# bebop/poly

Measured on AMD Instinct MI355X. Metric: mash.Sketch k-mers hashed/s, higher is better.
Workload: dtype u32

## Files before the change

### poly_amd/csrc/mash_sketch.hip

```cpp
#include <hip/hip_runtime.h>

#include <algorithm>

#include "common.h"
#include "host_pipeline.h"
#include "multi_device.h"
#include <memory>
#include <string>
#include <vector>

#ifndef PH_WPE
#define PH_WPE 6
#endif
#ifndef PH_CAPK
#define PH_CAPK 12u
#endif
#ifndef PH_ABL
#define PH_ABL 0
#endif
#ifndef PH_SEL_ATOMIC
#define PH_SEL_ATOMIC 0
#endif
#ifndef PH_BS_WIN
#define PH_BS_WIN 4
#endif
#ifndef PH_BS_U
#define PH_BS_U 4
#endif
#ifndef PH_SLAB_SIG
#define PH_SLAB_SIG 6u
#endif
#ifndef PH_SLAB_CW
#define PH_SLAB_CW 6u
#endif
#ifndef PH_SLAB_CF
#define PH_SLAB_CF 0u
#endif
#ifndef PH_SLAB_WPE
#define PH_SLAB_WPE 8
#endif

namespace polyhip {
namespace k1 {

constexpr int THREADS = 256;
constexpr int WAVES = THREADS / 64;
#ifndef PH_WTW
#define PH_WTW 512
#endif
constexpr int WTW = PH_WTW;
constexpr int TW = WTW * WAVES;
constexpr int GROUPS = WTW / (4 * 64);
constexpr int NB = 2048;
constexpr uint32_t MARK0 = 0xFFFFFFFFu, MARK1 = 0u;
constexpr int GBATCH = 32;
constexpr uint32_t WL_POSITIONAL = 0x80000000u;
constexpr uint32_t C1 = 0xcc9e2d51u, C2 = 0x1b873593u;

__device__ __forceinline__ uint32_t rotl32(uint32_t x, int r) { return (x << r) | (x >> (32 - r)); }

__device__ __forceinline__ uint32_t premix(uint32_t k)
{
    k *= C1;
    k = rotl32(k, 15);
    k *= C2;
    return k;
}

__device__ __forceinline__ uint32_t chain(uint32_t h) { return rotl32(h, 13) * 5u + 0xe6546b64u; }

__device__ __forceinline__ uint32_t fmix32(uint32_t h)
{
    h ^= h >> 16;
    h *= 0x85ebca6bu;
    h ^= h >> 13;
    h *= 0xc2b2ae35u;
    h ^= h >> 16;
    return h;
}

__device__ __forceinline__ uint32_t funnel_bytes(uint32_t hi, uint32_t lo, uint32_t sh)
{
    return __builtin_amdgcn_alignbyte(hi, lo, sh);
}

__device__ __forceinline__ uint32_t wave_incl_scan(uint32_t v)
{
    v += (uint32_t)__builtin_amdgcn_update_dpp(0, (int)v, 0x111, 0xF, 0xF, true);
    v += (uint32_t)__builtin_amdgcn_update_dpp(0, (int)v, 0x112, 0xF, 0xF, true);
    v += (uint32_t)__builtin_amdgcn_update_dpp(0, (int)v, 0x114, 0xF, 0xF, true);
    v += (uint32_t)__builtin_amdgcn_update_dpp(0, (int)v, 0x118, 0xF, 0xF, true);
    v += (uint32_t)__builtin_amdgcn_update_dpp(0, (int)v, 0x142, 0xA, 0xF, false);
    v += (uint32_t)__builtin_amdgcn_update_dpp(0, (int)v, 0x143, 0xC, 0xF, false);
    return v;
}

struct Smem {
    uint32_t *seqb;
    uint32_t *P;
    uint32_t *cand;
    uint32_t *binned;
    uint32_t *misc;
    uint32_t *lut;
    uint32_t *bins;
    uint32_t *biglist;
    uint32_t listcap;
};

constexpr uint32_t BIG_BIN = 32;
constexpr uint32_t BIG_LIST_CAP = 512;

template <class Bin, class Emit>
__device__ __attribute__((noinline)) void rank_big_bins(const uint32_t *__restrict__ binned, const Bin *__restrict__ bins,
                                              const uint32_t *__restrict__ biglist, uint32_t nbig, uint32_t s, Emit emit)
{
    const int lane = threadIdx.x & 63, wave = threadIdx.x >> 6;
    const uint64_t below = (1ull << lane) - 1ull;
    for (uint32_t q = wave; q < nbig; q += WAVES) {
        const uint32_t b = biglist[q];
        const uint32_t st = b ? bins[b - 1] : 0u, en = bins[b];
        uint32_t base = st, lastv = 0;
        bool first = true;
        while (base < s && base < en) {
            uint32_t m = 0xFFFFFFFFu;
            bool has = false;
            for (uint32_t x = st + lane; x < en; x += 64) {
                const uint32_t o = binned[x];
                if (first || o > lastv) {
                    m = min(m, o);
                    has = true;
                }
            }
            if (__ballot(has) == 0ull)
                break;
#pragma unroll
            for (int d = 32; d >= 1; d >>= 1)
                m = min(m, (uint32_t)__shfl_xor((int)m, d, 64));
            for (uint32_t x0 = st; x0 < en; x0 += 64) {
                const uint32_t x = x0 + lane;
                const bool eq = x < en && binned[x] == m;
                const uint64_t mask = __ballot(eq);
                const uint32_t pos = base + (uint32_t)__builtin_popcountll(mask & below);
                if (eq && pos < s)
                    emit(pos, m);
                base += (uint32_t)__builtin_popcountll(mask);
            }
            lastv = m;
            first = false;
        }
    }
}

template <class ForEach>
__device__ uint32_t bottom_s(const Smem &sm, uint32_t s, uint32_t tau, uint32_t binned_cap, bool keep_partial,
                             ForEach for_each)
{
    const int tid = threadIdx.x;
    uint32_t *bins = sm.P;
    const int sig = 32 - __builtin_clz(tau | 1u);
    const int shift = sig > 11 ? sig - 11 : 0;
    __syncthreads();

    for (int b = tid; b < NB; b += THREADS)
        bins[b] = 0;
    if (tid == 0)
        sm.misc[8] = 0;
    __syncthreads();
    for_each([&](uint32_t h) {
        if (h <= tau)
            atomicAdd(&bins[h >> shift], 1u);
    });
    __syncthreads();

    {
        uint32_t v[8], sum = 0;
#pragma unroll
        for (int i = 0; i < 8; ++i) {
            v[i] = bins[8 * tid + i];
            sum += v[i];
        }
        uint32_t incl = sum;
#pragma unroll
        for (int d = 1; d < 64; d <<= 1) {
            uint32_t t = __shfl_up(incl, d, 64);
            if ((tid & 63) >= d)
                incl += t;
        }
        if ((tid & 63) == 63)
            sm.misc[4 + (tid >> 6)] = incl;
        __syncthreads();
        uint32_t run = incl - sum;
        for (int w = 0; w < (tid >> 6); ++w)
            run += sm.misc[4 + w];
#pragma unroll
        for (int i = 0; i < 8; ++i) {
            bins[8 * tid + i] = run;
            run += v[i];
            if (v[i] > BIG_BIN) {
                const uint32_t slot = atomicAdd(&sm.misc[8], 1u);
                if (slot < BIG_LIST_CAP)
                    sm.seqb[slot] = (uint32_t)(8 * tid + i);
            }
        }
        if (tid == THREADS - 1)
            sm.misc[3] = run;
    }
    __syncthreads();
    const uint32_t T = sm.misc[3];
    if (T > binned_cap || (T < s && !keep_partial))
        return T;
    for_each([&](uint32_t h) {
        if (h <= tau)
            sm.binned[atomicAdd(&bins[h >> shift], 1u)] = h;
    });
    __syncthreads();
    if (T < s) {
        for (uint32_t j = tid; j < T; j += THREADS)
            sm.cand[j] = sm.binned[j];
        __syncthreads();
        if (tid == 0)
            sm.misc[0] = T;
        __syncthreads();
        return T;
    }
    const uint32_t nbig = sm.misc[8];
    const bool by_waves = nbig <= BIG_LIST_CAP;
    for (uint32_t j = tid; j < T; j += THREADS) {
        const uint32_t h = sm.binned[j];
        const uint32_t b = h >> shift;
        const uint32_t start = b ? bins[b - 1] : 0u;
        if (start >= s)
            continue;
        const uint32_t end = bins[b];
        if (by_waves && end - start > BIG_BIN)
            continue;
        uint32_t rank = 0;
        for (uint32_t x = start; x < end; ++x) {
            const uint32_t o = sm.binned[x];
            rank += (o < h) || (o == h && x < j);
        }
        const uint32_t pos = start + rank;
        if (pos < s)
            sm.cand[pos] = h;
    }
    if (by_waves && nbig)
        rank_big_bins(sm.binned, bins, sm.seqb, nbig, s, [cand = sm.cand](uint32_t pos, uint32_t h) { cand[pos] = h; });
    __syncthreads();
    if (tid == 0) {
        sm.misc[0] = s;
        sm.misc[1] = sm.cand[s - 1];
    }
    __syncthreads();
    return T;
}

__device__ __forceinline__ void wave_sync()
{
    asm volatile("" ::: "memory");
    __builtin_amdgcn_wave_barrier();
    asm volatile("" ::: "memory");
}

template <int KS> struct Stager {
    static constexpr int NI = KS > 0 ? ((WTW / 4 + KS / 4 + 2 + 3) + 63) / 64 : 1;
    uint32_t lo[NI], hi[NI];

    __device__ __forceinline__ static void fetch(const uint32_t *__restrict__ gdw, uint32_t gsh, int64_t gbytes,
                                                 int64_t gi, bool full, uint32_t &l, uint32_t &h)
    {
        if (PH_ABL == 6) {
            l = (uint32_t)gi * 0x9E3779B9u;
            h = l;
            return;
        }
        h = 0u;
        if (full) {
            l = gdw[gi];
            if (gsh)
                h = gdw[gi + 1];
        } else {
            l = (gi * 4 < gbytes) ? gdw[gi] : 0u;
            if (gsh)
                h = ((gi + 1) * 4 < gbytes) ? gdw[gi + 1] : 0u;
        }
    }

    __device__ __forceinline__ void load(const uint32_t *__restrict__ gdw, uint32_t gsh, int64_t gbytes, int64_t t0,
                                         uint32_t n_seq_dw, bool full)
    {
        if (KS > 0) {
            const int64_t dbase = t0 >> 2;
#pragma unroll
            for (int i = 0; i < NI; ++i) {
                const uint32_t d = (threadIdx.x & 63) + i * 64;
                if (d < n_seq_dw)
                    fetch(gdw, gsh, gbytes, dbase + d, full, lo[i], hi[i]);
            }
        }
    }

    __device__ __forceinline__ void store(uint32_t *__restrict__ seqb, const uint32_t *__restrict__ gdw, uint32_t gsh,
                                          int64_t gbytes, int64_t t0, uint32_t n_seq_dw, bool full)
    {
        if (KS > 0) {
#pragma unroll
            for (int i = 0; i < NI; ++i) {
                const uint32_t d = (threadIdx.x & 63) + i * 64;
                if (d < n_seq_dw)
                    seqb[d] = gsh ? funnel_bytes(hi[i], lo[i], gsh) : lo[i];
            }
        } else {
            const int64_t dbase = t0 >> 2;
            for (uint32_t d = threadIdx.x & 63; d < n_seq_dw; d += 64) {
                uint32_t l, h;
                fetch(gdw, gsh, gbytes, dbase + d, full, l, h);
                seqb[d] = gsh ? funnel_bytes(h, l, gsh) : l;
            }
        }
    }
};

template <int KS, class Emit>
__device__ __forceinline__ void tile_compute(const uint32_t *__restrict__ seqb, uint32_t *__restrict__ P,
                                             const uint32_t *__restrict__ lut, uint32_t k, Emit emit)
{
    const int lane = threadIdx.x & 63;
    const int nblk = (int)(k >> 2);
    const int tail = (int)(k & 3);
    const uint32_t tailmask = tail == 0 ? 0u : (0xFFFFFFFFu >> (32 - 8 * tail));

    {
        const int nq = (WTW >> 2) + nblk;
        for (int q = lane; q < (PH_ABL == 1 ? 0 : nq); q += 64) {
            const uint32_t d0 = seqb[q], d1 = seqb[q + 1];
            uint4 p;
            p.x = premix(d0);
            p.y = premix(funnel_bytes(d1, d0, 1));
            p.z = premix(funnel_bytes(d1, d0, 2));
            p.w = premix(funnel_bytes(d1, d0, 3));
            reinterpret_cast<uint4 *>(P)[q] = p;
        }
    }
    wave_sync();

    const uint4 *P4 = reinterpret_cast<const uint4 *>(P);
#pragma unroll
    for (int g = 0; g < GROUPS; ++g) {
        const int wq = lane + 64 * g;
        uint32_t h[4] = {0u, 0u, 0u, 0u};
        if (KS > 0) {
#pragma unroll
            for (int j = 0; j < (PH_ABL == 2 ? 1 : (KS >> 2)); ++j) {
                const uint4 p = P4[wq + j];
                h[0] = chain(h[0] ^ p.x);
                h[1] = chain(h[1] ^ p.y);
                h[2] = chain(h[2] ^ p.z);
                h[3] = chain(h[3] ^ p.w);
            }
        } else {
            for (int j = 0; j < nblk; ++j) {
                const uint4 p = P4[wq + j];
                h[0] = chain(h[0] ^ p.x);
                h[1] = chain(h[1] ^ p.y);
                h[2] = chain(h[2] ^ p.z);
                h[3] = chain(h[3] ^ p.w);
            }
        }
        if (PH_ABL == 3) {
        } else if (tail == 1) {
            const uint32_t tb = seqb[wq + nblk];
            h[0] ^= lut[tb & 0xFFu];
            h[1] ^= lut[(tb >> 8) & 0xFFu];
            h[2] ^= lut[(tb >> 16) & 0xFFu];
            h[3] ^= lut[tb >> 24];
        } else if (tail) {
            const uint32_t d0 = seqb[wq + nblk], d1 = seqb[wq + nblk + 1];
            h[0] ^= premix(d0 & tailmask) ^ k;
            h[1] ^= premix(funnel_bytes(d1, d0, 1) & tailmask) ^ k;
            h[2] ^= premix(funnel_bytes(d1, d0, 2) & tailmask) ^ k;
            h[3] ^= premix(funnel_bytes(d1, d0, 3) & tailmask) ^ k;
        } else {
#pragma unroll
            for (int c = 0; c < 4; ++c)
                h[c] ^= k;
        }
#pragma unroll
        for (int c = 0; c < 4; ++c)
            h[c] = PH_ABL == 3 ? h[c] : fmix32(h[c]);
        emit(4u * (uint32_t)wq, h);
    }
    wave_sync();
}

template <int KS, bool LOCKSTEP, class Before, class EmitFull, class EmitPart>
__device__ __forceinline__ void run_tiles(const Smem &sm, const uint32_t *__restrict__ gdw, uint32_t gsh,
                                          int64_t gbytes, int64_t nwin, uint32_t k, uint32_t n_seq_dw, uint32_t n_P_w,
                                          Before before, EmitFull emit_full, EmitPart emit_part)
{
    const int wave = threadIdx.x >> 6;
    uint32_t *seqb = sm.seqb + wave * n_seq_dw;
    uint32_t *P = sm.P + wave * n_P_w;
    const int64_t stage_bytes = (int64_t)n_seq_dw * 4 + 4;
    auto is_full = [&](int64_t t0) { return (nwin - t0) >= (int64_t)WTW && t0 + stage_bytes <= gbytes; };
    Stager<KS> st;
    const int64_t first = (int64_t)wave * WTW;
    if (first < nwin)
        st.load(gdw, gsh, gbytes, first, n_seq_dw, is_full(first));
    for (int64_t T0 = 0; T0 < nwin; T0 += TW) {
        if (LOCKSTEP)
            before(T0);
        const int64_t t0 = T0 + first;
        if (t0 >= nwin)
            continue;
        const bool full = is_full(t0);
        st.store(seqb, gdw, gsh, gbytes, t0, n_seq_dw, full);
        wave_sync();
        if (t0 + TW < nwin)
            st.load(gdw, gsh, gbytes, t0 + TW, n_seq_dw, is_full(t0 + TW));
        if (full) {
            tile_compute<KS>(seqb, P, sm.lut, k, [&](uint32_t w0, const uint32_t(&h)[4]) { emit_full(t0, w0, h, 4u); });
        } else {
            const uint32_t wl = (uint32_t)((nwin - t0) < (int64_t)WTW ? (nwin - t0) : (int64_t)WTW);
            tile_compute<KS>(seqb, P, sm.lut, k, [&](uint32_t w0, const uint32_t(&h)[4]) {
                emit_part(t0, w0, h, w0 >= wl ? 0u : (wl - w0 < 4u ? wl - w0 : 4u));
            });
        }
    }
}

__device__ __forceinline__ void append4(uint32_t *__restrict__ counter, uint32_t *__restrict__ cand, uint32_t cap,
                                        const uint32_t (&h)[4], uint32_t nvalid, uint32_t tau)
{
    bool a[4];
    uint64_t m[4];
    uint32_t cnt[4], total = 0;
#pragma unroll
    for (int c = 0; c < 4; ++c) {
        a[c] = (PH_ABL == 4 ? h[c] == 12345u : h[c] <= tau) && (uint32_t)c < nvalid;
        m[c] = __ballot(a[c]);
        cnt[c] = (uint32_t)__popcll(m[c]);
        total += cnt[c];
    }
    if (total == 0)
        return;
    uint32_t base = 0;
    if ((threadIdx.x & 63) == 0)
        base = atomicAdd(counter, total);
    base = __builtin_amdgcn_readfirstlane(base);
#pragma unroll
    for (int c = 0; c < 4; ++c) {
        if (a[c]) {
            const uint32_t idx = base + __builtin_amdgcn_mbcnt_hi((uint32_t)(m[c] >> 32),
                                                                  __builtin_amdgcn_mbcnt_lo((uint32_t)m[c], 0u));
            if (idx < cap)
                cand[idx] = h[c];
        }
        base += cnt[c];
    }
}

constexpr int BSU = PH_BS_U;
constexpr uint32_t BS_MARGIN = (PH_BS_WIN + 3u) & ~3u;
#define BS_SYNC()              \
    do {                       \
        if (PH_ABL != 21)      \
            __syncthreads();   \
    } while (0)
template <bool FIN>
__device__ void bottom_s_fast(const Smem &sm, uint32_t s, uint32_t tau, uint32_t C, uint32_t nbf_log2,
                              uint32_t *__restrict__ outp, const uint32_t *__restrict__ src, uint32_t first,
                              uint32_t step, uint32_t cnt)
{
    const int tid = threadIdx.x;
    auto fin = [](uint32_t h) { return FIN ? h ^ (h >> 16) : h; };
    uint32_t *bins = sm.bins;
    const uint16_t *bins16 = reinterpret_cast<const uint16_t *>(bins);
    const int sig = 32 - __builtin_clz(tau | 1u);
    const int shift = sig > (int)nbf_log2 ? sig - (int)nbf_log2 : 0;
    auto one = [](uint32_t b) { return 1u << ((b & 1u) << 4); };
    const bool wide = nbf_log2 == 11u;
    if (wide)
        reinterpret_cast<uint4 *>(bins)[tid] = make_uint4(0, 0, 0, 0);
    else
        reinterpret_cast<uint2 *>(bins)[tid] = make_uint2(0, 0);
    if (tid == 0)
        sm.misc[8] = 0;
    if (PH_BS_WIN) {
        if (tid < PH_BS_WIN)
            sm.binned[-1 - tid] = 0u;
        else if (tid < 2 * PH_BS_WIN)
            sm.binned[C + (uint32_t)tid - PH_BS_WIN] = 0xFFFFFFFFu;
    }
    BS_SYNC();
    for (uint32_t i0 = first; i0 < cnt; i0 += BSU * step) {
        uint32_t h[BSU];
#pragma unroll
        for (int u = 0; u < BSU; ++u)
            h[u] = i0 + u * step < cnt ? fin(src[i0 + u * step]) : 0u;
#pragma unroll
        for (int u = 0; u < BSU; ++u)
            if (i0 + u * step < cnt) {
                const uint32_t b = h[u] >> shift;
                atomicAdd(&bins[b >> 1], one(b));
            }
    }
    BS_SYNC();
    {
        uint32_t w[4];
        if (wide) {
            const uint4 t = reinterpret_cast<const uint4 *>(bins)[tid];
            w[0] = t.x, w[1] = t.y, w[2] = t.z, w[3] = t.w;
        } else {
            const uint2 t = reinterpret_cast<const uint2 *>(bins)[tid];
            w[0] = t.x, w[1] = t.y, w[2] = 0u, w[3] = 0u;
        }
        uint32_t c[8], sum = 0;
#pragma unroll
        for (int i = 0; i < 8; ++i) {
            c[i] = (w[i >> 1] >> (16 * (i & 1))) & 0xFFFFu;
            sum += c[i];
        }
        const uint32_t incl = wave_incl_scan(sum);
        if ((tid & 63) == 63)
            sm.misc[4 + (tid >> 6)] = incl;
        BS_SYNC();
        uint32_t run = incl - sum;
        for (int w8 = 0; w8 < (tid >> 6); ++w8)
            run += sm.misc[4 + w8];
        const uint32_t b0 = (uint32_t)tid << (wide ? 3 : 2);
#pragma unroll
        for (int i = 0; i < 4; ++i) {
            w[i] = run | ((run + c[2 * i]) << 16);
            run += c[2 * i] + c[2 * i + 1];
        }
        if (wide)
            reinterpret_cast<uint4 *>(bins)[tid] = make_uint4(w[0], w[1], w[2], w[3]);
        else
            reinterpret_cast<uint2 *>(bins)[tid] = make_uint2(w[0], w[1]);
        if (max(max(max(c[0], c[1]), max(c[2], c[3])), max(max(c[4], c[5]), max(c[6], c[7]))) > BIG_BIN) {
#pragma unroll
            for (int i = 0; i < 8; ++i)
                if (c[i] > BIG_BIN) {
                    const uint32_t slot = atomicAdd(&sm.misc[8], 1u);
                    if (slot < sm.listcap)
                        sm.biglist[slot] = b0 + (uint32_t)i;
                }
        }
    }
    BS_SYNC();
    for (uint32_t i0 = first; i0 < cnt; i0 += BSU * step) {
        uint32_t h[BSU], at[BSU];
#pragma unroll
        for (int u = 0; u < BSU; ++u)
            h[u] = i0 + u * step < cnt ? fin(src[i0 + u * step]) : 0u;
#pragma unroll
        for (int u = 0; u < BSU; ++u)
            if (i0 + u * step < cnt) {
                const uint32_t b = h[u] >> shift;
                at[u] = (atomicAdd(&bins[b >> 1], one(b)) >> ((b & 1u) << 4)) & 0xFFFFu;
            }
#pragma unroll
        for (int u = 0; u < BSU; ++u)
            if (i0 + u * step < cnt)
                sm.binned[at[u]] = h[u];
    }
    BS_SYNC();
    const uint32_t nbig = sm.misc[8];
    const bool by_waves = nbig <= sm.listcap;
    auto rank_in_bin = [&](uint32_t j, uint32_t hv) {
        const uint32_t b = hv >> shift;
        const uint32_t start = b ? bins16[b - 1] : 0u, end = bins16[b];
        if (start >= s || (by_waves && end - start > BIG_BIN))
            return;
        uint32_t pos = start;
        for (uint32_t x = start; x < end; ++x) {
            const uint32_t o = sm.binned[x];
            pos += (o < hv) || (o == hv && x < j);
        }
        if (pos < s)
            outp[pos] = hv;
    };
#if PH_BS_WIN
    if (PH_ABL != 22) {
        const uint32_t lim = 1u << shift;
        for (uint32_t j = tid; j < C; j += THREADS) {
            const uint32_t *__restrict__ w = sm.binned + j;
            const uint32_t hv = w[0];
            uint32_t pos = j;
            bool far;
            {
                uint32_t l[PH_BS_WIN], r[PH_BS_WIN];
#pragma unroll
                for (int d = 0; d < PH_BS_WIN; ++d) {
                    l[d] = w[-1 - d];
                    r[d] = w[1 + d];
                }
#pragma unroll
                for (int d = 0; d < PH_BS_WIN; ++d) {
                    pos -= l[d] > hv ? 1u : 0u;
                    pos += r[d] < hv ? 1u : 0u;
                }
                far = ((l[PH_BS_WIN - 1] ^ hv) < lim) | ((r[PH_BS_WIN - 1] ^ hv) < lim);
            }
            if (__builtin_expect(far, 0))
                rank_in_bin(j, hv);
            else if (pos < s)
                outp[pos] = hv;
        }
    }
#else
    for (uint32_t j = tid; j < C; j += THREADS)
        rank_in_bin(j, sm.binned[j]);
#endif
    if (by_waves && nbig)
        rank_big_bins(sm.binned, bins16, sm.biglist, nbig, s, [outp](uint32_t pos, uint32_t hv) { outp[pos] = hv; });
}

struct ReadView {
    const uint32_t *gdw;
    uint32_t gsh;
    int64_t gbytes, nwin;
};

__device__ __forceinline__ ReadView view(const uint8_t *__restrict__ seqs, const uint64_t *__restrict__ offs,
                                         uint64_t r, uint32_t k)
{
    ReadView v;
    const uint64_t o0 = offs[r], o1 = offs[r + 1];
    const int64_t n = (int64_t)(o1 - o0);
    v.nwin = n - (int64_t)k;
    v.gsh = (uint32_t)((uintptr_t)(seqs + o0) & 3);
    v.gdw = reinterpret_cast<const uint32_t *>(seqs + o0 - v.gsh);
    v.gbytes = n + v.gsh;
    return v;
}

template <int KS>
__global__ __launch_bounds__(THREADS) __attribute__((amdgpu_waves_per_eu(PH_WPE, 8))) void sketch_fast_kernel(const uint8_t *__restrict__ seqs,
                                                             const uint64_t *__restrict__ offs, uint64_t nseq,
                                                             uint32_t k_rt, uint32_t s, uint32_t *__restrict__ out,
                                                             uint32_t n_seq_dw, uint32_t n_P_w, uint32_t n_P,
                                                             uint32_t capf, uint32_t nbf_log2)
{
    extern __shared__ __attribute__((aligned(16))) uint32_t smem_raw[];
    Smem sm;
    sm.seqb = smem_raw;
    sm.P = sm.seqb + WAVES * n_seq_dw;
    sm.cand = sm.P + n_P;
    sm.binned = sm.cand + capf + BS_MARGIN;
    sm.misc = sm.binned + capf + BS_MARGIN;
    sm.lut = sm.misc + 16;
    sm.bins = sm.P;
    sm.biglist = sm.seqb;
    sm.listcap = BIG_LIST_CAP;

    const uint32_t k = KS > 0 ? (uint32_t)KS : k_rt;
    const int tid = threadIdx.x;
    sm.lut[tid] = premix((uint32_t)tid) ^ k;
    auto nothing = [](int64_t) {};

    for (uint64_t r = blockIdx.x; r < nseq; r += gridDim.x) {
        const ReadView rv = view(seqs, offs, r, k);
        if (rv.nwin <= 0)
            continue;
        uint32_t *__restrict__ outp = out + r * (uint64_t)s;

        if (rv.nwin < (int64_t)s) {
            __syncthreads();
            auto put = [&](int64_t t0, uint32_t w0, const uint32_t(&h)[4], uint32_t nvalid) {
#pragma unroll
                for (int c = 0; c < 4; ++c)
                    if ((uint32_t)c < nvalid)
                        outp[t0 + w0 + c] = h[c];
            };
            run_tiles<KS, false>(sm, rv.gdw, rv.gsh, rv.gbytes, rv.nwin, k, n_seq_dw, n_P_w, nothing, put, put);
            continue;
        }

        uint32_t tau0 = 0xFFFFFFFFu;
        {
            const uint64_t target = (uint64_t)s + 6ull * (uint64_t)__builtin_sqrtf((float)s) + 16ull;
            if ((int64_t)target < rv.nwin)
                tau0 = (uint32_t)((target << 32) / (uint64_t)rv.nwin);
        }
        bool ok = tau0 != 0xFFFFFFFFu || rv.nwin <= (int64_t)capf;
        __syncthreads();
        if (tid == 0)
            sm.misc[0] = 0;
        __syncthreads();
        uint32_t C = 0;
        if (ok) {
            auto keep = [&](int64_t, uint32_t, const uint32_t(&h)[4], uint32_t nvalid) {
                append4(&sm.misc[0], sm.cand, capf, h, nvalid, tau0);
            };
            run_tiles<KS, false>(sm, rv.gdw, rv.gsh, rv.gbytes, rv.nwin, k, n_seq_dw, n_P_w, nothing, keep, keep);
            __syncthreads();
            C = sm.misc[0];
            ok = C >= s && C <= capf;
        }
        if (ok) {
            if (PH_ABL == 5) {
                for (uint32_t i = tid; i < s; i += THREADS)
                    outp[i] = sm.cand[i];
            } else {
                bottom_s_fast<false>(sm, s, tau0, C, nbf_log2, outp, sm.cand, (uint32_t)tid, THREADS, C);
            }
        } else if (tid == 0) {
            outp[0] = MARK0;
            outp[1] = MARK1;
        }
    }
}

template <int KS> struct Slabs {
    static constexpr int NBLK = KS >> 2, TAIL = KS & 3;
    static constexpr int DUPD = NBLK + 2;
    const uint32_t *__restrict__ gdw;
    uint32_t gsh;
    uint32_t *__restrict__ seqb;
    uint32_t *__restrict__ P;
    const uint32_t *__restrict__ lut;
    int lane;

    uint32_t u_inside;
    uint32_t gb32;
    __device__ __forceinline__ void gload(uint32_t u, uint32_t &lo, uint32_t &hi) const
    {
        const uint32_t *__restrict__ slab = gdw + (uint64_t)u * 64;
        hi = 0u;
        if (__builtin_expect(u < u_inside, 1)) {
            lo = slab[lane];
            if (gsh)
                hi = slab[lane + 1];
        } else {
            const int left = (int)(gb32 - u * 256u);
            lo = lane * 4 < left ? slab[lane] : 0u;
            if (gsh)
                hi = (lane + 1) * 4 < left ? slab[lane + 1] : 0u;
        }
    }

    template <int PAR> __device__ __forceinline__ void stage(uint32_t lo, uint32_t hi) const
    {
        const uint32_t v = gsh ? funnel_bytes(hi, lo, gsh) : lo;
        seqb[1 + 64 * PAR + lane] = v;
        if (PAR == 0) {
            if (lane < DUPD)
                seqb[129 + lane] = v;
        } else if (lane == 63) {
            seqb[0] = v;
        }
    }

    template <int PAR> __device__ __forceinline__ void premix_unit() const
    {
        const uint32_t d0 = seqb[64 * PAR + lane], d1 = seqb[64 * PAR + lane + 1];
        uint4 p;
        p.x = premix(d0);
        p.y = premix(funnel_bytes(d1, d0, 1));
        p.z = premix(funnel_bytes(d1, d0, 2));
        p.w = premix(funnel_bytes(d1, d0, 3));
        uint4 *P4 = reinterpret_cast<uint4 *>(P);
        if (PAR == 0) {
            P4[(lane + 127) & 127] = p;
            if (lane >= 1 && lane <= NBLK)
                P4[127 + lane] = p;
        } else {
            P4[63 + lane] = p;
        }
    }

    template <int PAR> __device__ __forceinline__ void hash(uint32_t (&h)[4]) const
    {
        const uint4 *b = reinterpret_cast<const uint4 *>(P) + 64 * PAR + lane;
        h[0] = h[1] = h[2] = h[3] = 0u;
#pragma unroll
        for (int j = 0; j < (PH_ABL == 16 ? 1 : NBLK); ++j) {
            const uint4 p = b[j];
            h[0] = chain(h[0] ^ p.x);
            h[1] = chain(h[1] ^ p.y);
            h[2] = chain(h[2] ^ p.z);
            h[3] = chain(h[3] ^ p.w);
        }
        const uint32_t *t = seqb + 1 + 64 * PAR + lane + NBLK;
        if (TAIL == 1) {
            const uint32_t tb = t[0];
            uint32_t off[4];
            const uint32_t two = 2u;
            asm("v_lshlrev_b32_sdwa %0, %1, %2 dst_sel:DWORD dst_unused:UNUSED_PAD src0_sel:DWORD src1_sel:BYTE_0" : "=v"(off[0]) : "v"(two), "v"(tb));
            asm("v_lshlrev_b32_sdwa %0, %1, %2 dst_sel:DWORD dst_unused:UNUSED_PAD src0_sel:DWORD src1_sel:BYTE_1" : "=v"(off[1]) : "v"(two), "v"(tb));
            asm("v_lshlrev_b32_sdwa %0, %1, %2 dst_sel:DWORD dst_unused:UNUSED_PAD src0_sel:DWORD src1_sel:BYTE_2" : "=v"(off[2]) : "v"(two), "v"(tb));
            asm("v_lshlrev_b32_sdwa %0, %1, %2 dst_sel:DWORD dst_unused:UNUSED_PAD src0_sel:DWORD src1_sel:BYTE_3" : "=v"(off[3]) : "v"(two), "v"(tb));
#pragma unroll
            for (int c = 0; c < 4; ++c)
                h[c] ^= *reinterpret_cast<const __attribute__((address_space(3))) uint32_t *>((uintptr_t)off[c]);
        } else if (TAIL) {
            constexpr uint32_t tailmask = 0xFFFFFFFFu >> (32 - 8 * (TAIL ? TAIL : 1));
            const uint32_t d0 = t[0], d1 = t[1];
            h[0] ^= premix(d0 & tailmask) ^ (uint32_t)KS;
            h[1] ^= premix(funnel_bytes(d1, d0, 1) & tailmask) ^ (uint32_t)KS;
            h[2] ^= premix(funnel_bytes(d1, d0, 2) & tailmask) ^ (uint32_t)KS;
            h[3] ^= premix(funnel_bytes(d1, d0, 3) & tailmask) ^ (uint32_t)KS;
        } else {
#pragma unroll
            for (int c = 0; c < 4; ++c)
                h[c] ^= (uint32_t)KS;
        }
#pragma unroll
        for (int c = 0; c < 4; ++c) {
            uint32_t x = h[c];
            if (PH_ABL != 17) {
                x ^= x >> 16;
                x *= 0x85ebca6bu;
                x ^= x >> 13;
            }
            x *= 0xc2b2ae35u;
            h[c] = x;
        }
    }
};

template <bool PARTIAL>
__device__ __forceinline__ void append_own(uint32_t *__restrict__ seg, uint32_t capw, uint32_t &cnt, const uint32_t (&h)[4],
                                           uint32_t nvalid, uint32_t tauq)
{
    bool a[4];
    uint64_t m[4];
    uint32_t n[4], total = 0;
#pragma unroll
    for (int c = 0; c < 4; ++c) {
        a[c] = h[c] <= tauq && (!PARTIAL || (uint32_t)c < nvalid);
        m[c] = __ballot(a[c]);
        n[c] = (uint32_t)__popcll(m[c]);
        total += n[c];
    }
    uint32_t base = __builtin_amdgcn_readfirstlane(cnt);
    cnt = base + total;
#if PH_SEL_ATOMIC
    {
        uint32_t *ctr = seg + capw;
        uint32_t slot[4];
#pragma unroll
        for (int c = 0; c < 4; ++c)
            if (a[c])
                slot[c] = atomicInc(ctr, capw - 1u);
#pragma unroll
        for (int c = 0; c < 4; ++c)
            if (a[c])
                seg[slot[c]] = h[c];
        return;
    }
#endif
    if (cnt <= capw) {
#pragma unroll
        for (int c = 0; c < 4; ++c) {
            uint32_t *__restrict__ at = seg + base;
            if (a[c])
                at[__builtin_amdgcn_mbcnt_hi((uint32_t)(m[c] >> 32), __builtin_amdgcn_mbcnt_lo((uint32_t)m[c], 0u))] = h[c];
            base += n[c];
        }
    }
}

template <int KS>
__device__ __forceinline__ uint32_t run_slabs(const Smem &sm, const ReadView &rv, uint32_t n_seq_dw, uint32_t n_P_w,
                                              uint32_t *__restrict__ seg, uint32_t capw, uint32_t tauq)
{
    const int wave = __builtin_amdgcn_readfirstlane(threadIdx.x >> 6);
    Slabs<KS> S;
    S.gdw = rv.gdw;
    S.gsh = rv.gsh;
    S.seqb = sm.seqb + wave * n_seq_dw;
    S.P = sm.P + wave * n_P_w;
    S.lut = sm.lut;
    S.lane = threadIdx.x & 63;
    const uint32_t nslab = (uint32_t)((rv.nwin + 255) >> 8);
    const uint32_t spw = (nslab + WAVES - 1) / WAVES;
    const uint32_t a = (uint32_t)wave * spw, b = a + spw < nslab ? a + spw : nslab;
    S.u_inside = rv.gbytes >= 65 * 4 ? (uint32_t)(((rv.gbytes >> 2) - 65) >> 6) + 1u : 0u;
    S.gb32 = (uint32_t)rv.gbytes;
    const uint32_t nfull = (uint32_t)(rv.nwin >> 8), rem = (uint32_t)rv.nwin & 255u;
    uint32_t cnt = 0;
#if PH_SEL_ATOMIC
    capw -= 1u;
    if (S.lane == 0)
        seg[capw] = 0u;
#endif
    if (a >= b)
        return cnt;
    uint32_t l1, h1;
    S.gload(a, l1, h1);
    if (a & 1) {
        S.template stage<1>(l1, h1);
        wave_sync();
        S.gload(a + 1, l1, h1);
        S.template premix_unit<1>();
    } else {
        S.template stage<0>(l1, h1);
        wave_sync();
        S.gload(a + 1, l1, h1);
        S.template premix_unit<0>();
    }
    for (uint32_t i = a; i < b; ++i) {
        uint32_t h[4];
        if (i & 1) {
            S.template stage<0>(l1, h1);
            wave_sync();
            S.gload(i + 2, l1, h1);
            if (PH_ABL != 15)
                S.template premix_unit<0>();
            wave_sync();
            S.template hash<1>(h);
        } else {
            S.template stage<1>(l1, h1);
            wave_sync();
            S.gload(i + 2, l1, h1);
            if (PH_ABL != 15)
                S.template premix_unit<1>();
            wave_sync();
            S.template hash<0>(h);
        }
        if (PH_ABL == 11) {
            if ((h[0] ^ h[1] ^ h[2] ^ h[3]) == 0x12345u)
                seg[0] = h[0];
        } else if (__builtin_expect(i < nfull, 1)) {
            append_own<false>(seg, capw, cnt, h, 4u, tauq);
        } else {
            const int mine = (int)rem - 4 * S.lane;
            append_own<true>(seg, capw, cnt, h, mine <= 0 ? 0u : (mine < 4 ? (uint32_t)mine : 4u), tauq);
        }
        wave_sync();
    }
    return cnt;
}

template <int KS>
__global__ __launch_bounds__(THREADS) __attribute__((amdgpu_waves_per_eu(PH_SLAB_WPE, 8))) void sketch_slab_kernel(
    const uint8_t *__restrict__ seqs, const uint64_t *__restrict__ offs, uint64_t nseq, uint32_t s, uint32_t *__restrict__ out,
    uint32_t n_seq_dw, uint32_t n_P_w, uint32_t n_span, uint32_t capw, uint32_t capf, uint32_t nbf_log2)
{
    extern __shared__ __attribute__((aligned(16))) uint32_t smem_raw[];
    Smem sm;
    sm.lut = smem_raw;
    sm.seqb = smem_raw + 256;
    sm.P = sm.seqb + WAVES * n_seq_dw;
    sm.bins = sm.seqb;
    sm.binned = sm.bins + ((1u << nbf_log2) >> 1) + BS_MARGIN;
    sm.biglist = sm.binned + capf + BS_MARGIN;
    sm.listcap = (uint32_t)(sm.seqb + n_span - sm.biglist);
    sm.misc = sm.seqb + n_span;
    sm.cand = sm.misc + 16;
    constexpr uint32_t k = (uint32_t)KS;
    const int tid = threadIdx.x, wave = __builtin_amdgcn_readfirstlane(tid >> 6);
    sm.lut[tid] = premix((uint32_t)tid) ^ k;
    uint32_t *seg = sm.cand + wave * capw;

    for (uint64_t r = blockIdx.x; r < nseq; r += gridDim.x) {
        const ReadView rv = view(seqs, offs, r, k);
        if (rv.nwin <= 0)
            continue;
        uint32_t *__restrict__ outp = out + r * (uint64_t)s;
        if (rv.nwin < (int64_t)s)
            continue;
        uint32_t tauq = 0xFFFFFFFFu;
        {
            const uint64_t target = (uint64_t)s + (uint64_t)PH_SLAB_SIG * (uint64_t)__builtin_sqrtf((float)s) + 16ull;
            if ((int64_t)target < rv.nwin)
                tauq = (uint32_t)((target << 32) / (uint64_t)rv.nwin) | 0xFFFFu;
        }
        __syncthreads();
        const uint32_t cw = PH_ABL == 14 ? tauq >> 31 : run_slabs<KS>(sm, rv, n_seq_dw, n_P_w, seg, capw, tauq);
        if ((tid & 63) == 0)
            sm.misc[10 + wave] = cw;
        __syncthreads();
        if (PH_ABL == 11 || PH_ABL == 12 || PH_ABL == 14) {
            if (sm.misc[10] + sm.misc[11] + sm.misc[12] + sm.misc[13] == 0xFFFFFFF0u)
                outp[0] = cw;
            continue;
        }
        const uint32_t c0 = sm.misc[10], c1 = sm.misc[11], c2 = sm.misc[12], c3 = sm.misc[13];
        const uint32_t C = c0 + c1 + c2 + c3;
        const bool ok = max(max(c0, c1), max(c2, c3)) <= capw - (PH_SEL_ATOMIC ? 1u : 0u) && C >= s && C <= capf;
        if (ok)
            bottom_s_fast<true>(sm, s, tauq, C, nbf_log2, outp, seg, (uint32_t)(tid & 63), 64u, cw);
        else if (tid == 0) {
            outp[0] = MARK0;
            outp[1] = MARK1;
        }
    }
}

template <int KS>
__global__ __launch_bounds__(THREADS) void sketch_general_kernel(const uint8_t *__restrict__ seqs,
                                                                const uint64_t *__restrict__ offs, uint32_t k_rt,
                                                                uint32_t s, uint32_t *__restrict__ out,
                                                                uint32_t n_seq_dw, uint32_t n_P_w, uint32_t n_P,
                                                                uint32_t cap, uint64_t nseq, int take_positional)
{
    extern __shared__ __attribute__((aligned(16))) uint32_t smem_raw[];
    Smem sm;
    sm.seqb = smem_raw;
    sm.P = sm.seqb + WAVES * n_seq_dw;
    sm.cand = sm.P + n_P;
    sm.binned = sm.cand + cap;
    sm.misc = sm.binned + cap;
    sm.lut = sm.misc + 16;
    __shared__ uint32_t wl[GBATCH];
    __shared__ uint32_t nwl;

    const uint32_t k = KS > 0 ? (uint32_t)KS : k_rt;
    const int tid = threadIdx.x;
    sm.lut[tid] = premix((uint32_t)tid) ^ k;

    for (uint64_t base = (uint64_t)blockIdx.x * GBATCH; base < nseq; base += (uint64_t)gridDim.x * GBATCH) {
        __syncthreads();
        if (tid == 0)
            nwl = 0;
        __syncthreads();
        {
            const uint64_t r = base + tid;
            if (tid < GBATCH && r < nseq) {
                const int64_t nwin = (int64_t)(offs[r + 1] - offs[r]) - (int64_t)k;
                uint32_t need = 0;
                if (nwin >= (int64_t)s) {
                    const uint32_t *row = out + r * (uint64_t)s;
                    if (row[0] == MARK0 && row[1] == MARK1)
                        need = 1;
                } else if (nwin > 0 && take_positional) {
                    need = 2;
                }
                if (need)
                    wl[atomicAdd(&nwl, 1u)] = (uint32_t)tid | (need == 2 ? WL_POSITIONAL : 0u);
            }
        }
        __syncthreads();
        const uint32_t nredo = nwl;
    for (uint32_t q = 0; q < nredo; ++q) {
        const uint32_t entry = wl[q];
        const uint64_t r = base + (entry & ~WL_POSITIONAL);
        const ReadView rv = view(seqs, offs, r, k);
        uint32_t *__restrict__ outp = out + r * (uint64_t)s;
        __syncthreads();
        if (entry & WL_POSITIONAL) {
            auto put = [&](int64_t t0, uint32_t w0, const uint32_t(&h)[4], uint32_t nvalid) {
#pragma unroll
                for (int c = 0; c < 4; ++c)
                    if ((uint32_t)c < nvalid)
                        outp[t0 + w0 + c] = h[c];
            };
            run_tiles<KS, false>(sm, rv.gdw, rv.gsh, rv.gbytes, rv.nwin, k, n_seq_dw, n_P_w, [](int64_t) {}, put, put);
            continue;
        }
        if (tid == 0) {
            sm.misc[0] = 0;
            sm.misc[1] = 0xFFFFFFFFu;
        }
        __syncthreads();
        auto shrink_shared = [&]() {
            const uint32_t C = sm.misc[0];
            bottom_s(sm, s, sm.misc[1], cap, true, [&](auto f) {
                for (uint32_t i = tid; i < C; i += THREADS)
                    f(sm.cand[i]);
            });
        };
        auto append = [&](int64_t, uint32_t, const uint32_t(&h)[4], uint32_t nvalid) {
            append4(&sm.misc[0], sm.cand, cap, h, nvalid, sm.misc[1]);
        };
        run_tiles<KS, true>(
            sm, rv.gdw, rv.gsh, rv.gbytes, rv.nwin, k, n_seq_dw, n_P_w,
            [&](int64_t) {
                __syncthreads();
                const bool room = sm.misc[0] + (uint32_t)TW <= cap;
                __syncthreads();
                if (!room)
                    shrink_shared();
            },
            append, append);
        __syncthreads();
        shrink_shared();
        for (uint32_t i = tid; i < s; i += THREADS)
            outp[i] = sm.cand[i];
    }
    }
}


constexpr uint32_t WIDE_ROUND = 4 * THREADS;

__device__ __forceinline__ uint32_t murmur3_window(const uint8_t *__restrict__ p, uint32_t k)
{
    uint32_t h = 0;
    const uint32_t nblk = k >> 2;
    for (uint32_t j = 0; j < nblk; ++j) {
        uint32_t w;
        __builtin_memcpy(&w, p + 4 * (size_t)j, 4);
        h = chain(h ^ premix(w));
    }
    const uint8_t *t = p + 4 * (size_t)nblk;
    uint32_t w = 0;
    switch (k & 3u) {
    case 3: w ^= (uint32_t)t[2] << 16; [[fallthrough]];
    case 2: w ^= (uint32_t)t[1] << 8; [[fallthrough]];
    case 1: w ^= (uint32_t)t[0]; h ^= premix(w); break;
    default: break;
    }
    return fmix32(h ^ k);
}

__global__ __launch_bounds__(THREADS) void sketch_wide_kernel(const uint8_t *__restrict__ seqs,
                                                             const uint64_t *__restrict__ offs, uint64_t nseq, uint32_t k,
                                                             uint32_t s, uint32_t *__restrict__ out,
                                                             uint32_t *__restrict__ scratch, uint32_t cap)
{
    __shared__ uint32_t bins[NB];
    __shared__ uint32_t biglist[BIG_LIST_CAP];
    __shared__ uint32_t misc[16];
    Smem sm;
    sm.seqb = biglist;
    sm.P = bins;
    sm.cand = scratch + (size_t)blockIdx.x * 2 * cap;
    sm.binned = sm.cand + cap;
    sm.misc = misc;
    sm.lut = nullptr;
    const int tid = threadIdx.x;
    for (uint64_t r = blockIdx.x; r < nseq; r += gridDim.x) {
        const uint64_t o0 = offs[r];
        const int64_t nwin = (int64_t)(offs[r + 1] - o0) - (int64_t)k;
        if (nwin <= 0)
            continue;
        const uint8_t *__restrict__ sp = seqs + o0;
        uint32_t *__restrict__ outp = out + r * (uint64_t)s;
        if (nwin < (int64_t)s) {
            for (int64_t w = tid; w < nwin; w += THREADS)
                outp[w] = murmur3_window(sp + w, k);
            continue;
        }
        __syncthreads();
        if (tid == 0) {
            misc[0] = 0;
            misc[1] = 0xFFFFFFFFu;
        }
        __syncthreads();
        auto shrink = [&]() {
            const uint32_t C = misc[0];
            bottom_s(sm, s, misc[1], cap, true, [&](auto f) {
                for (uint32_t i = tid; i < C; i += THREADS)
                    f(sm.cand[i]);
            });
        };
        for (int64_t base = 0; base < nwin; base += WIDE_ROUND) {
            __syncthreads();
            const bool room = misc[0] + WIDE_ROUND <= cap;
            __syncthreads();
            if (!room)
                shrink();
            const uint32_t tau = misc[1];
#pragma unroll
            for (int c = 0; c < 4; ++c) {
                const int64_t w = base + c * THREADS + tid;
                if (w < nwin) {
                    const uint32_t h = murmur3_window(sp + w, k);
                    if (h <= tau)
                        sm.cand[atomicAdd(&misc[0], 1u)] = h;
                }
            }
        }
        __syncthreads();
        shrink();
        for (uint32_t i = tid; i < s; i += THREADS)
            outp[i] = sm.cand[i];
    }
}

__global__ __launch_bounds__(THREADS) void sketch_tiny_kernel(const uint8_t *__restrict__ seqs,
                                                             const uint64_t *__restrict__ offs, uint64_t nseq, uint32_t k,
                                                             uint32_t s, uint32_t *__restrict__ out,
                                                             unsigned long long *__restrict__ first_panic)
{
    const int tid = threadIdx.x;
    for (uint64_t r = blockIdx.x; r < nseq; r += gridDim.x) {
        const uint64_t o0 = offs[r];
        const int64_t nwin = (int64_t)(offs[r + 1] - o0) - (int64_t)k;
        if (nwin <= 0)
            continue;
        if (s == 0) {
            if (tid == 0)
                atomicMin(first_panic, (unsigned long long)r);
            continue;
        }
        const uint8_t *__restrict__ sp = seqs + o0;
        const uint32_t h0 = murmur3_window(sp, k);
        bool under = false;
        for (int64_t w = 1 + tid; w < nwin && !under; w += THREADS)
            under = murmur3_window(sp + w, k) < h0;
        if (__syncthreads_or(under ? 1 : 0)) {
            if (tid == 0)
                atomicMin(first_panic, (unsigned long long)r);
        } else if (tid == 0) {
            out[r] = h0;
        }
    }
}

struct Launch {
    uint32_t n_seq_dw, n_P_w, n_P, n_P_fast, nbf_log2, nbf_log2_slab, capf, cap, capw, capf_slab, n_span;
    size_t smem_fast, smem_general, smem_slab;
};

static Launch plan(uint32_t k, uint32_t s)
{
    Launch L;
    const uint32_t nblk = k / 4;
    L.n_seq_dw = ((WTW / 4 + nblk + 2) + 3u) & ~3u;
    L.n_P_w = WTW + 4 * nblk;
    L.n_P = WAVES * L.n_P_w;
    L.n_P_fast = L.n_P < 1024u ? 1024u : L.n_P;
    L.nbf_log2 = L.n_P_fast >= 2048u ? 11u : 10u;
    if (L.n_P < (uint32_t)NB)
        L.n_P = NB;
    const uint32_t s4 = (s + 3u) & ~3u;
    uint32_t rt = 1;
    while ((uint64_t)rt * rt < s)
        ++rt;
    L.capf = (s4 + PH_CAPK * rt + 64u + 63u) & ~63u;
    L.cap = s4 + TW + 64u;
    const size_t common = (size_t)WAVES * L.n_seq_dw + L.n_P + 16 + 256;
    L.smem_fast = ((size_t)WAVES * L.n_seq_dw + L.n_P_fast + 16 + 256 + 2 * (size_t)L.capf + 2 * BS_MARGIN) * 4;
    if (PH_ABL == 7)
        L.smem_fast = 70 * 1024;
    L.smem_general = (common + 2 * (size_t)L.cap) * 4;
    {
        const uint32_t target = s + PH_SLAB_SIG * rt + 16u;
        const uint32_t exp_w = (target + WAVES - 1) / WAVES;
        uint32_t rw = 1;
        while ((uint64_t)rw * rw < exp_w)
            ++rw;
        L.capw = (exp_w + PH_SLAB_CW * rw + 8u + 63u) & ~63u;
        L.capf_slab = PH_SLAB_CF ? ((target + PH_SLAB_CF * rt + 8u + 63u) & ~63u) : L.capf;
    }
    L.nbf_log2_slab = 11;
    {
        const uint32_t rings = WAVES * (L.n_seq_dw + L.n_P_w);
        const uint32_t sorted = ((1u << L.nbf_log2_slab) >> 1) + L.capf_slab + 2 * BS_MARGIN + L.capf_slab / (BIG_BIN + 1) + 1;
        L.n_span = rings > sorted ? rings : sorted;
    }
    L.smem_slab = ((size_t)256 + L.n_span + 16 + (size_t)WAVES * L.capw) * 4;
#ifdef PH_LDS_PAD
    L.smem_slab += PH_LDS_PAD;
#endif
    return L;
}

static unsigned persistent_grid(size_t smem, uint64_t n)
{
    const uint64_t per_cu = std::max<uint64_t>(1, std::min<uint64_t>(8, (160 * 1024) / std::max<size_t>(smem, 1)));
    return (unsigned)std::min<uint64_t>(n, 256 * per_cu * 4);
}

template <int KS>
static int launch(const uint8_t *d_seqs, const uint64_t *d_offs, uint64_t n, uint32_t k, uint32_t s,
                  uint32_t *d_out, const Launch &L, hipStream_t st)
{
    auto general = sketch_general_kernel<KS>;
    PH_HIP(hipFuncSetAttribute(reinterpret_cast<const void *>(general), hipFuncAttributeMaxDynamicSharedMemorySize,
                               (int)L.smem_general));
    bool slabs = false;
    if constexpr (KS > 0) {
        slabs = !env_is("POLYHIP_K1_SLABS", '0') && L.smem_slab <= 64 * 1024;
        if (slabs) {
            auto slab = sketch_slab_kernel<KS>;
            PH_HIP(hipFuncSetAttribute(reinterpret_cast<const void *>(slab), hipFuncAttributeMaxDynamicSharedMemorySize,
                                       (int)L.smem_slab));
            hipLaunchKernelGGL(slab, dim3(persistent_grid(L.smem_slab, n)), dim3(THREADS), L.smem_slab, st, d_seqs, d_offs, n, s,
                               d_out, L.n_seq_dw, L.n_P_w, L.n_span, L.capw, L.capf_slab, L.nbf_log2_slab);
        }
    }
    if (!slabs) {
        auto fast = sketch_fast_kernel<KS>;
        PH_HIP(hipFuncSetAttribute(reinterpret_cast<const void *>(fast), hipFuncAttributeMaxDynamicSharedMemorySize,
                                   (int)L.smem_fast));
        hipLaunchKernelGGL(fast, dim3(persistent_grid(L.smem_fast, n)), dim3(THREADS), L.smem_fast, st, d_seqs, d_offs, n,
                           k, s, d_out, L.n_seq_dw, L.n_P_w, L.n_P_fast, L.capf, L.nbf_log2);
    }
    PH_HIP(hipGetLastError());
    const unsigned ggrid = (unsigned)std::min<uint64_t>((n + GBATCH - 1) / GBATCH, persistent_grid(L.smem_general, n));
    hipLaunchKernelGGL(general, dim3(ggrid), dim3(THREADS), L.smem_general, st, d_seqs, d_offs, k, s, d_out, L.n_seq_dw,
                       L.n_P_w, L.n_P, L.cap, n, slabs ? 1 : 0);
// ... 227 lines not shown
```

Measured before the change: 865.6 billion.

## Scatter only bins up to the s-th boundary bin and pre-zero bins early

The bottom-s selection now finds the bin that contains the s-th smallest hash during the prefix scan. It scatters and ranks only the candidates in bins up to that one, so work beyond the cutoff is skipped. The first BSR hashes are kept in registers across both passes to avoid reloading them. In the slab path, the bin histogram is zeroed before the existing barrier, in regions that alias the per-wave sequence and P buffers, which removes one barrier. The zeroing regions are computed from the buffer sizes, which could leave bins uncovered if those sizes do not span the bin array.

```diff
diff --git a/poly_amd/csrc/mash_sketch.hip b/poly_amd/csrc/mash_sketch.hip
--- a/poly_amd/csrc/mash_sketch.hip
+++ b/poly_amd/csrc/mash_sketch.hip
@@ -24,8 +24,8 @@
 #ifndef PH_BS_WIN
 #define PH_BS_WIN 4
 #endif
-#ifndef PH_BS_U
-#define PH_BS_U 4
+#ifndef PH_BS_R
+#define PH_BS_R 6
 #endif
 #ifndef PH_SLAB_SIG
 #define PH_SLAB_SIG 6u
@@ -459,17 +459,11 @@
     }
 }
 
-constexpr int BSU = PH_BS_U;
+constexpr int BSR = PH_BS_R;
 constexpr uint32_t BS_MARGIN = (PH_BS_WIN + 3u) & ~3u;
-#define BS_SYNC()              \
-    do {                       \
-        if (PH_ABL != 21)      \
-            __syncthreads();   \
-    } while (0)
-template <bool FIN>
-__device__ void bottom_s_fast(const Smem &sm, uint32_t s, uint32_t tau, uint32_t C, uint32_t nbf_log2,
-                              uint32_t *__restrict__ outp, const uint32_t *__restrict__ src, uint32_t first,
-                              uint32_t step, uint32_t cnt)
+template <bool FIN, bool ZEROED>
+__device__ void bottom_s_fast(const Smem &sm, uint32_t s, uint32_t tau, uint32_t nbf_log2, uint32_t *__restrict__ outp,
+                              const uint32_t *__restrict__ src, uint32_t first, uint32_t step, uint32_t cnt)
 {
     const int tid = threadIdx.x;
     auto fin = [](uint32_t h) { return FIN ? h ^ (h >> 16) : h; };
@@ -479,32 +473,29 @@
     const int shift = sig > (int)nbf_log2 ? sig - (int)nbf_log2 : 0;
     auto one = [](uint32_t b) { return 1u << ((b & 1u) << 4); };
     const bool wide = nbf_log2 == 11u;
-    if (wide)
-        reinterpret_cast<uint4 *>(bins)[tid] = make_uint4(0, 0, 0, 0);
-    else
-        reinterpret_cast<uint2 *>(bins)[tid] = make_uint2(0, 0);
-    if (tid == 0)
-        sm.misc[8] = 0;
-    if (PH_BS_WIN) {
-        if (tid < PH_BS_WIN)
-            sm.binned[-1 - tid] = 0u;
-        else if (tid < 2 * PH_BS_WIN)
-            sm.binned[C + (uint32_t)tid - PH_BS_WIN] = 0xFFFFFFFFu;
-    }
-    BS_SYNC();
-    for (uint32_t i0 = first; i0 < cnt; i0 += BSU * step) {
-        uint32_t h[BSU];
-#pragma unroll
-        for (int u = 0; u < BSU; ++u)
-            h[u] = i0 + u * step < cnt ? fin(src[i0 + u * step]) : 0u;
-#pragma unroll
-        for (int u = 0; u < BSU; ++u)
-            if (i0 + u * step < cnt) {
-                const uint32_t b = h[u] >> shift;
-                atomicAdd(&bins[b >> 1], one(b));
-            }
-    }
-    BS_SYNC();
+    if (!ZEROED) {
+        if (wide)
+            reinterpret_cast<uint4 *>(bins)[tid] = make_uint4(0, 0, 0, 0);
+        else
+            reinterpret_cast<uint2 *>(bins)[tid] = make_uint2(0, 0);
+        if (tid == 0)
+            sm.misc[8] = 0;
+        __syncthreads();
+    }
+    uint32_t h[BSR];
+#pragma unroll
+    for (int u = 0; u < BSR; ++u)
+        h[u] = first + u * step < cnt ? fin(src[first + u * step]) : 0u;
+    auto bn = [&](int u) { return h[u] >> shift; };
+#pragma unroll
+    for (int u = 0; u < BSR; ++u)
+        if (first + u * step < cnt)
+            atomicAdd(&bins[bn(u) >> 1], one(bn(u)));
+    for (uint32_t i = first + BSR * step; i < cnt; i += step) {
+        const uint32_t b = fin(src[i]) >> shift;
+        atomicAdd(&bins[b >> 1], one(b));
+    }
+    __syncthreads();
     {
         uint32_t w[4];
         if (wide) {
@@ -523,11 +514,30 @@
         const uint32_t incl = wave_incl_scan(sum);
         if ((tid & 63) == 63)
             sm.misc[4 + (tid >> 6)] = incl;
-        BS_SYNC();
+        __syncthreads();
         uint32_t run = incl - sum;
         for (int w8 = 0; w8 < (tid >> 6); ++w8)
             run += sm.misc[4 + w8];
         const uint32_t b0 = (uint32_t)tid << (wide ? 3 : 2);
+        if (run < s && s <= run + sum) {
+            uint32_t st = run, bstar = 0, E = 0;
+            bool found = false;
+#pragma unroll
+            for (int i = 0; i < 8; ++i) {
+                if (!found && st + c[i] >= s) {
+                    bstar = b0 + (uint32_t)i;
+                    E = st + c[i];
+                    found = true;
+                }
+                st += c[i];
+            }
+            sm.misc[14] = bstar;
+            sm.misc[15] = E;
+            for (int d = 0; d < PH_BS_WIN; ++d) {
+                sm.binned[-1 - d] = 0u;
+                sm.binned[E + d] = 0xFFFFFFFFu;
+            }
+        }
 #pragma unroll
         for (int i = 0; i < 4; ++i) {
             w[i] = run | ((run + c[2 * i]) << 16);
@@ -547,24 +557,31 @@
                 }
         }
     }
-    BS_SYNC();
-    for (uint32_t i0 = first; i0 < cnt; i0 += BSU * step) {
-        uint32_t h[BSU], at[BSU];
-#pragma unroll
-        for (int u = 0; u < BSU; ++u)
-            h[u] = i0 + u * step < cnt ? fin(src[i0 + u * step]) : 0u;
-#pragma unroll
-        for (int u = 0; u < BSU; ++u)
-            if (i0 + u * step < cnt) {
-                const uint32_t b = h[u] >> shift;
-                at[u] = (atomicAdd(&bins[b >> 1], one(b)) >> ((b & 1u) << 4)) & 0xFFFFu;
-            }
-#pragma unroll
-        for (int u = 0; u < BSU; ++u)
-            if (i0 + u * step < cnt)
-                sm.binned[at[u]] = h[u];
-    }
-    BS_SYNC();
+    __syncthreads();
+    if (PH_ABL == 23)
+        return;
+    const uint32_t bstar = sm.misc[14], E = sm.misc[15];
+    {
+        constexpr int BSG = 4;
+#pragma unroll
+        for (int g = 0; g < BSR; g += BSG) {
+            uint32_t at[BSG];
+#pragma unroll
+            for (int u = g; u < g + BSG && u < BSR; ++u)
+                if (first + u * step < cnt && bn(u) <= bstar)
+                    at[u - g] = (atomicAdd(&bins[bn(u) >> 1], one(bn(u))) >> ((bn(u) & 1u) << 4)) & 0xFFFFu;
+#pragma unroll
+            for (int u = g; u < g + BSG && u < BSR; ++u)
+                if (first + u * step < cnt && bn(u) <= bstar)
+                    sm.binned[at[u - g]] = h[u];
+        }
+        for (uint32_t i = first + BSR * step; i < cnt; i += step) {
+            const uint32_t hv = fin(src[i]), b = hv >> shift;
+            if (b <= bstar)
+                sm.binned[(atomicAdd(&bins[b >> 1], one(b)) >> ((b & 1u) << 4)) & 0xFFFFu] = hv;
+        }
+    }
+    __syncthreads();
     const uint32_t nbig = sm.misc[8];
     const bool by_waves = nbig <= sm.listcap;
     auto rank_in_bin = [&](uint32_t j, uint32_t hv) {
@@ -583,7 +600,7 @@
 #if PH_BS_WIN
     if (PH_ABL != 22) {
         const uint32_t lim = 1u << shift;
-        for (uint32_t j = tid; j < C; j += THREADS) {
+        for (uint32_t j = tid; j < E; j += THREADS) {
             const uint32_t *__restrict__ w = sm.binned + j;
             const uint32_t hv = w[0];
             uint32_t pos = j;
@@ -609,7 +626,7 @@
         }
     }
 #else
-    for (uint32_t j = tid; j < C; j += THREADS)
+    for (uint32_t j = tid; j < E; j += THREADS)
         rank_in_bin(j, sm.binned[j]);
 #endif
     if (by_waves && nbig)
@@ -703,7 +720,7 @@
                 for (uint32_t i = tid; i < s; i += THREADS)
                     outp[i] = sm.cand[i];
             } else {
-                bottom_s_fast<false>(sm, s, tau0, C, nbf_log2, outp, sm.cand, (uint32_t)tid, THREADS, C);
+                bottom_s_fast<false, false>(sm, s, tau0, nbf_log2, outp, sm.cand, (uint32_t)tid, THREADS, C);
             }
         } else if (tid == 0) {
             outp[0] = MARK0;
@@ -972,6 +989,20 @@
         const uint32_t cw = PH_ABL == 14 ? tauq >> 31 : run_slabs<KS>(sm, rv, n_seq_dw, n_P_w, seg, capw, tauq);
         if ((tid & 63) == 0)
             sm.misc[10 + wave] = cw;
+        {
+            uint4 *b4 = reinterpret_cast<uint4 *>(sm.bins);
+            uint32_t lane = tid & 63;
+            asm volatile("" : "+v"(lane));
+            const uint32_t nbq = 1u << (nbf_log2 - 3);
+            const uint32_t s0 = wave * (n_seq_dw >> 2), s1 = min(s0 + (n_seq_dw >> 2), nbq);
+            const uint32_t p0 = WAVES * (n_seq_dw >> 2) + wave * (n_P_w >> 2), p1 = min(p0 + (n_P_w >> 2), nbq);
+            for (uint32_t q = s0 + lane; q < s1; q += 64)
+                b4[q] = make_uint4(0, 0, 0, 0);
+            for (uint32_t q = p0 + lane; q < p1; q += 64)
+                b4[q] = make_uint4(0, 0, 0, 0);
+            if (tid == 0)
+                sm.misc[8] = 0;
+        }
         __syncthreads();
         if (PH_ABL == 11 || PH_ABL == 12 || PH_ABL == 14) {
             if (sm.misc[10] + sm.misc[11] + sm.misc[12] + sm.misc[13] == 0xFFFFFFF0u)
@@ -982,7 +1013,7 @@
         const uint32_t C = c0 + c1 + c2 + c3;
         const bool ok = max(max(c0, c1), max(c2, c3)) <= capw - (PH_SEL_ATOMIC ? 1u : 0u) && C >= s && C <= capf;
         if (ok)
-            bottom_s_fast<true>(sm, s, tauq, C, nbf_log2, outp, seg, (uint32_t)(tid & 63), 64u, cw);
+            bottom_s_fast<true, true>(sm, s, tauq, nbf_log2, outp, seg, (uint32_t)(tid & 63), 64u, cw);
         else if (tid == 0) {
             outp[0] = MARK0;
             outp[1] = MARK1;
```

Result: no change. 871.8 billion (median of 6 runs) (+0.7%).
